# floswald/SMM.jl

Hardware: AMD Instinct MI355X
Metric: chain-evals/sec (whole node), serialNormal 2p/2m, 4096 chains x 200 iters (higher is better)
Workload: dtype f64

## Files before the change

### smm.jl_amd/csrc/smm_lookahead.hpp

```cpp
#pragma once
__global__ void k_pregen_rng(const KParams P, const int t0, const int W, double* __restrict__ rb) {
    const int N = P.N, np = P.np, TR = P.rb_tries;
    const int Q = (np + 1) / 2;
    const uint32_t per_iter = (uint32_t)TR * (uint32_t)Q * (uint32_t)N;
    const uint32_t i = blockIdx.x * blockDim.x + threadIdx.x;
    if (i >= per_iter) return;
    const int q = (int)(i % (uint32_t)Q);
    const uint32_t rest = i / (uint32_t)Q;
    const int r = (int)(rest % (uint32_t)TR);
    const int c = (int)(rest / (uint32_t)TR);
    const int w = (int)blockIdx.y;
    const int t = t0 + w;
    const uint32_t gc = (uint32_t)(P.offset + c);
    double* blk = rb + ((size_t)w * N + c) * P.RBW;
    if (t > 1) {
        double z0, z1 = 0.0;
        if (P.user_ntab) {
            const size_t base = (((size_t)(t - 1) * TR + r) * np) * N + c;
            z0 = P.user_ntab[base + (size_t)(2 * q) * N];
            if (2 * q + 1 < np) z1 = P.user_ntab[base + (size_t)(2 * q + 1) * N];
        } else {
            rng_prop_normal2(P.seed, gc, (uint32_t)t, (uint32_t)r, (uint32_t)q, z0, z1);
        }
        blk[1 + r * np + 2 * q] = z0;
        if (2 * q + 1 < np) blk[1 + r * np + 2 * q + 1] = z1;
    }
    if (r == 0 && q == 0) blk[0] = P.user_utab ? P.user_utab[(size_t)(t - 1) * N + c] : rng_u(P.seed, gc, (uint32_t)t);
}

__global__ __launch_bounds__(XWG) void k_exch_plan(const KParams P, const int t0, unsigned long long* __restrict__ plan,
                                                   double* __restrict__ plan_mi, uint32_t* __restrict__ lv_pairs,
                                                   double* __restrict__ lv_mi, uint32_t* __restrict__ lv_off,
                                                   uint32_t* __restrict__ lv_pairs_p, uint32_t* __restrict__ lv_offp) {
    extern __shared__ __attribute__((aligned(16))) unsigned char xsm[];
    const int tid = threadIdx.x, lane = tid & 63, wave = tid >> 6;
    const int t = t0 + blockIdx.x;
    const int Ng = P.Ng, K = P.plan_K;
    uint32_t* cnt = (uint32_t*)xsm;
    uint32_t* ep = cnt + Ng + 2;
    uint16_t* pi = (uint16_t*)(ep + 2 * K);
    uint16_t* pj = pi + K;
    uint32_t* wsum = (uint32_t*)(pj + K);
    unsigned long long* out = plan + (size_t)blockIdx.x * K;
    double* out_mi = plan_mi + (size_t)blockIdx.x * K;

    if (P.ts && blockIdx.x == 0 && tid == 0) P.ts[(size_t)8 * 60000 + 80] = wall_clock64();
    for (int c = tid; c < Ng; c += XWG) cnt[c] = 0;
    if (P.pairtab) {
        for (int q = tid; q < K; q += XWG) {
            pi[q] = (uint16_t)P.pairtab[((size_t)(t - 1) * K + q) * 2];
            pj[q] = (uint16_t)P.pairtab[((size_t)(t - 1) * K + q) * 2 + 1];
        }
    } else {
        PairPerm pp;
        pp.init(P.seed, (uint32_t)t, (uint64_t)Ng * (uint64_t)(Ng - 1) / 2);
        for (int q = tid; q < K; q += XWG) {
            int32_t i, j;
            pair_unrank(pp.eval((uint64_t)q), i, j);
            pi[q] = (uint16_t)i;
            pj[q] = (uint16_t)j;
        }
    }
    __syncthreads();
    if (P.ts && blockIdx.x == 0 && tid == 0) P.ts[(size_t)8 * 60000 + 81] = wall_clock64();
    for (int q = tid; q < K; q += XWG) {
        atomicAdd(&cnt[pi[q]], 1u);
        atomicAdd(&cnt[pj[q]], 1u);
    }
    __syncthreads();
    {
        constexpr int PER = XLDS_MAX / XWG;
        const int per = (Ng + XWG - 1) / XWG;
        const int c0 = tid * per;
        uint32_t loc[PER];
        uint32_t sum = 0;
#pragma unroll
        for (int u = 0; u < PER; ++u) {
            const int c = c0 + u;
            const uint32_t v = (u < per && c < Ng) ? cnt[c] : 0u;
            loc[u] = sum;
            sum += v;
        }
        uint32_t incl = sum;
#pragma unroll
        for (int off = 1; off < 64; off <<= 1) {
            const uint32_t o = __shfl_up(incl, off, 64);
            if (lane >= off) incl += o;
        }
        if (lane == 63) wsum[wave] = incl;
        __syncthreads();
        uint32_t base = 0;
        for (int w = 0; w < wave; ++w) base += wsum[w];
        const uint32_t excl = base + incl - sum;
#pragma unroll
        for (int u = 0; u < PER; ++u) {
            const int c = c0 + u;
            if (u < per && c < Ng) cnt[c] = excl + loc[u];
        }
    }
    __syncthreads();
    for (int q = tid; q < K; q += XWG) {
        ep[atomicAdd(&cnt[pi[q]], 1u)] = (uint32_t)q;
        ep[atomicAdd(&cnt[pj[q]], 1u)] = (uint32_t)q;
    }
    __syncthreads();
    constexpr int MAXPP = XLDS_MAX / XWG;
    uint16_t rri[MAXPP], rrj[MAXPP];
#pragma unroll
    for (int m = 0; m < MAXPP; ++m) {
        const int q = tid + m * XWG;
        rri[m] = 0; rrj[m] = 0;
        if (q < K) {
            const uint32_t i = pi[q], j = pj[q];
            uint32_t b = i ? cnt[i - 1] : 0u, e = cnt[i], ri = 0, rj = 0;
            for (uint32_t x = b; x < e; ++x) ri += (ep[x] < (uint32_t)q) ? 1u : 0u;
            b = j ? cnt[j - 1] : 0u; e = cnt[j];
            for (uint32_t x = b; x < e; ++x) rj += (ep[x] < (uint32_t)q) ? 1u : 0u;
            out[q] = (unsigned long long)i | ((unsigned long long)j << 16) | ((unsigned long long)ri << 32) |
                     ((unsigned long long)rj << 48);
            out_mi[q] = P.min_improve_g[i];
            rri[m] = (uint16_t)ri; rrj[m] = (uint16_t)rj;
        }
    }
    __syncthreads();
    if (P.ts && blockIdx.x == 0 && tid == 0) P.ts[(size_t)8 * 60000 + 82] = wall_clock64();
#pragma unroll
    for (int m = 0; m < MAXPP; ++m) {
        const int q = tid + m * XWG;
        if (q < K) {
            const uint32_t i = pi[q], j = pj[q];
            ep[(i ? cnt[i - 1] : 0u) + rri[m]] = (uint32_t)q;
            ep[(j ? cnt[j - 1] : 0u) + rrj[m]] = (uint32_t)q;
        }
    }
    __syncthreads();
    int prei[MAXPP], prej[MAXPP];
    bool lasti[MAXPP], lastj[MAXPP];
#pragma unroll
    for (int m = 0; m < MAXPP; ++m) {
        const int q = tid + m * XWG;
        prei[m] = -1; prej[m] = -1; lasti[m] = false; lastj[m] = false;
        if (q < K) {
            const uint32_t i = pi[q], j = pj[q];
            if (rri[m]) prei[m] = (int)ep[(i ? cnt[i - 1] : 0u) + rri[m] - 1];
            if (rrj[m]) prej[m] = (int)ep[(j ? cnt[j - 1] : 0u) + rrj[m] - 1];
            lasti[m] = (i ? cnt[i - 1] : 0u) + rri[m] + 1u == cnt[i];
            lastj[m] = (j ? cnt[j - 1] : 0u) + rrj[m] + 1u == cnt[j];
        }
    }
    __syncthreads();
    uint16_t* lvl = (uint16_t*)ep;
    uint16_t* lvl_b = lvl + K;
    uint32_t* lhist = cnt;
    for (int q = tid; q < K; q += XWG) { lvl[q] = 0; lvl_b[q] = 0; }
    __syncthreads();
    {
        uint16_t own[MAXPP];
#pragma unroll
        for (int m = 0; m < MAXPP; ++m) own[m] = 0;
        const uint16_t* cur = lvl;
        uint16_t* nxt = lvl_b;
        int changed = 1;
        while (changed) {
            int mine = 0;
#pragma unroll
            for (int m = 0; m < MAXPP; ++m) {
                const int q = tid + m * XWG;
                if (q < K) {
                    const uint32_t a = prei[m] >= 0 ? cur[prei[m]] : 0u, b = prej[m] >= 0 ? cur[prej[m]] : 0u;
                    const bool known = (prei[m] < 0 || a) && (prej[m] < 0 || b);
                    const uint16_t nl = known ? (uint16_t)(1u + (a > b ? a : b)) : (uint16_t)0;
                    if (nl != own[m]) mine = 1;
                    own[m] = nl;
                    nxt[q] = nl;
                }
            }
            changed = __syncthreads_or(mine);
            const uint16_t* x = cur; cur = nxt; nxt = (uint16_t*)x;
        }
    }
    if (P.ts && blockIdx.x == 0 && tid == 0) P.ts[(size_t)8 * 60000 + 83] = wall_clock64();
    for (int c = tid; c < Ng + 2; c += XWG) lhist[c] = 0;
    __syncthreads();
    for (int q = tid; q < K; q += XWG) atomicAdd(&lhist[lvl[q]], 1u);
    __syncthreads();
    uint32_t* wsum2 = wsum + 16;
    __shared__ uint32_t s_nlev;
    if (tid == 0) s_nlev = 0;
    __syncthreads();
    {
        uint32_t mx = 0;
        for (int q = tid; q < K; q += XWG) mx = lvl[q] > mx ? lvl[q] : mx;
        atomicMax(&s_nlev, mx);
    }
    __syncthreads();
    const int nlev = (int)s_nlev;
    {
        constexpr int PER = XLDS_MAX / XWG + 1;
        const int n = nlev + 1;
        const int per = (n + XWG - 1) / XWG;
        const int c0 = tid * per;
        uint32_t loc[PER];
        uint32_t sum = 0;
#pragma unroll
        for (int u = 0; u < PER; ++u) {
            const int c = c0 + u;
            const uint32_t v = (u < per && c < n) ? lhist[c] : 0u;
            loc[u] = sum;
            sum += v;
        }
        uint32_t incl = sum;
#pragma unroll
        for (int off = 1; off < 64; off <<= 1) {
            const uint32_t o = __shfl_up(incl, off, 64);
            if (lane >= off) incl += o;
        }
        if (lane == 63) wsum2[wave] = incl;
        __syncthreads();
        uint32_t base = 0;
        for (int w = 0; w < wave; ++w) base += wsum2[w];
        const uint32_t excl = base + incl - sum;
#pragma unroll
        for (int u = 0; u < PER; ++u) {
            const int c = c0 + u;
            if (u < per && c < n) lhist[c] = excl + loc[u];
        }
    }
    __syncthreads();
    uint32_t* o_off = lv_off + (size_t)blockIdx.x * (K + 2);
    for (int l = tid; l < nlev; l += XWG) o_off[l] = (l + 2 <= nlev) ? lhist[l + 2] : (uint32_t)K;
    if (tid == 0) o_off[K + 1] = (uint32_t)nlev;
    __shared__ uint32_t s_lst[LV_MAXLEV + 2], s_pst[LV_MAXLEV + 2];
    const bool lean = lv_pairs_p != nullptr && nlev <= LV_MAXLEV;
    uint32_t* o_pp = lv_pairs_p ? lv_pairs_p + (size_t)blockIdx.x * P.plan_Kp : nullptr;
    if (lv_offp && tid == 0) {
        uint32_t* o = lv_offp + (size_t)blockIdx.x * LV_OFFP;
        o[33] = (uint32_t)nlev; o[34] = lean ? 1u : 0u;
        if (lean) {
            uint32_t acc = 0;
            for (int c = 1; c <= nlev; ++c) {
                s_lst[c] = lhist[c]; s_pst[c] = acc; o[c - 1] = acc;
                acc += ((c + 1 <= nlev ? lhist[c + 1] : (uint32_t)K) - lhist[c] + 63u) & ~63u;
            }
            s_pst[nlev + 1] = acc; o[nlev] = acc;
        }
    }
    __syncthreads();
    const uint32_t sc8 = (uint32_t)P.lean_unit;
    if (lean) {
        const uint32_t Ng4 = (uint32_t)((Ng + 3) & ~3);
        const uint32_t dummy = P.lean_wide ? (sc8 * Ng4) * 0x10001u : (sc8 * Ng4) | ((sc8 * (Ng4 + 1u)) << 16);
        for (uint32_t q = tid; q < s_pst[nlev + 1]; q += XWG) o_pp[q] = dummy;
    }
    __syncthreads();
    uint32_t* o_pairs = lv_pairs + (size_t)blockIdx.x * K;
    double* o_mi = lv_mi + (size_t)blockIdx.x * K;
    uint16_t ci[MAXPP], cj[MAXPP], lvq[MAXPP];
#pragma unroll
    for (int m = 0; m < MAXPP; ++m) {
        const int q = tid + m * XWG;
        ci[m] = 0; cj[m] = 0; lvq[m] = 0;
        if (q < K) {
            const uint32_t lv = lvl[q];
            const uint32_t pos = atomicAdd(&lhist[lv], 1u);
            const uint32_t i = pi[q], j = pj[q];
            o_pairs[pos] = i | (j << 16);
            o_mi[pos] = P.min_improve_g[i];
            if (lean) o_pp[s_pst[lv] + (pos - s_lst[lv])] = (sc8 * i) | ((sc8 * j) << 16);
            ci[m] = (uint16_t)i; cj[m] = (uint16_t)j; lvq[m] = (uint16_t)lv;
        }
    }
    if (P.ts && blockIdx.x == 0 && tid == 0) P.ts[(size_t)8 * 60000 + 84] = wall_clock64();
    if (P.cone_ok == nullptr) return;
    const int tiles = P.cone_tiles;
    uint32_t* o_ok = (uint32_t*)P.cone_ok + blockIdx.x;
    if (!lean) {
        if (tid == 0) *o_ok = 0u;
        return;
    }
    const int LS = nlev + 1;
    int wpp = (int)(((size_t)150 * 1024) / ((size_t)K * 4 + (size_t)32 * LS * 4 + 32 * 4));
    if (wpp > (tiles + 31) / 32) wpp = (tiles + 31) / 32;
    if (wpp < 1) { if (tid == 0) *o_ok = 0u; return; }
    __shared__ uint32_t s_bad;
    if (tid == 0) s_bad = 0u;
    uint32_t* need = (uint32_t*)xsm;
    uint32_t* lcnt = need + (size_t)K * wpp;
    uint32_t* gcnt = lcnt + (size_t)32 * wpp * LS;
    uint16_t* o_gl = P.cone_gather ? P.cone_gather + (size_t)blockIdx.x * tiles * CONE_GCAP : nullptr;
    uint32_t* o_hdr = (uint32_t*)P.cone_hdr + (size_t)blockIdx.x * tiles * CONE_HDRW;
    uint32_t* o_cp = (uint32_t*)P.cone_pairs + (size_t)blockIdx.x * tiles * (CONE_LEVELS * 64);
    const uint32_t ct = (uint32_t)P.cone_ct;
    for (int b0 = 0; b0 < tiles; b0 += 32 * wpp) {
        const int nb = min(32 * wpp, tiles - b0);
        __syncthreads();
        for (int x = tid; x < K * wpp + 32 * wpp * LS + 32 * wpp; x += XWG) need[x] = 0u;
        __syncthreads();
        auto seed = [&](const uint32_t c, const int q) {
            const uint32_t b = (c - (uint32_t)P.offset) / ct - (uint32_t)b0;
            if (b < (uint32_t)nb) atomicOr(&need[(size_t)q * wpp + (b >> 5)], 1u << (b & 31u));
        };
#pragma unroll
        for (int m = 0; m < MAXPP; ++m) {
            const int q = tid + m * XWG;
            if (q < K) {
                if (lasti[m]) seed(ci[m], q);
                if (lastj[m]) seed(cj[m], q);
            }
        }
        if (P.ts && blockIdx.x == 0 && tid == 0) P.ts[(size_t)8 * 60000 + 85] = wall_clock64();
        __syncthreads();
        for (int l = nlev; l >= 2; --l) {
#pragma unroll
            for (int m = 0; m < MAXPP; ++m) {
                const int q = tid + m * XWG;
                if (q < K && lvq[m] == l) {
                    uint32_t* ri = prei[m] >= 0 ? &need[(size_t)prei[m] * wpp] : nullptr;
                    uint32_t* rj = prej[m] >= 0 ? &need[(size_t)prej[m] * wpp] : nullptr;
                    if ((wpp & 3) == 0) {
                        for (int w = 0; w < wpp; w += 8) {
                            const uint4 v0 = *(const uint4*)&need[(size_t)q * wpp + w];
                            const uint4 v1 = w + 4 < wpp ? *(const uint4*)&need[(size_t)q * wpp + w + 4] : make_uint4(0u, 0u, 0u, 0u);
                            const uint32_t v[8] = {v0.x, v0.y, v0.z, v0.w, v1.x, v1.y, v1.z, v1.w};
#pragma unroll
                            for (int x = 0; x < 8; ++x)
                                if (v[x]) {
                                    if (ri) atomicOr(&ri[w + x], v[x]);
                                    if (rj) atomicOr(&rj[w + x], v[x]);
                                }
                        }
                    } else
                        for (int w = 0; w < wpp; ++w) {
                            const uint32_t v = need[(size_t)q * wpp + w];
                            if (v) {
                                if (ri) atomicOr(&ri[w], v);
                                if (rj) atomicOr(&rj[w], v);
                            }
                        }
                }
            }
            __syncthreads();
        }
        if (P.ts && blockIdx.x == 0 && tid == 0) P.ts[(size_t)8 * 60000 + 86] = wall_clock64();
#pragma unroll
        for (int m = 0; m < MAXPP; ++m) {
            const int q = tid + m * XWG;
            if (q < K)
                for (int w = 0; w < wpp; ++w) {
                    uint32_t bits = need[(size_t)q * wpp + w];
                    while (bits) {
                        const uint32_t b = (uint32_t)w * 32u + (uint32_t)__builtin_ctz(bits);
                        bits &= bits - 1u;
                        atomicAdd(&lcnt[b * LS + lvq[m]], 1u);
                    }
                }
        }
        __syncthreads();
        if (P.ts && blockIdx.x == 0 && tid == 0) P.ts[(size_t)8 * 60000 + 87] = wall_clock64();
        for (int b = tid; b < nb; b += XWG) {
            uint32_t sub = 0;
            uint32_t hw[CONE_HDRW];
#pragma unroll
            for (int x = 0; x < CONE_HDRW; ++x) hw[x] = 0u;
            for (int l = 1; l <= nlev; ++l) {
                const uint32_t n = lcnt[b * LS + l];
                lcnt[b * LS + l] = sub * 64u;
                for (uint32_t x = 0; x < n; x += 64u, ++sub)
                    if (sub < (uint32_t)CONE_LEVELS) {
                        const uint32_t cnt_s = n - x < 64u ? n - x : 64u;
#pragma unroll
                        for (int y = 0; y < CONE_LEVELS / 4; ++y)
                            if ((int)(sub >> 2) == y) hw[1 + y] |= cnt_s << (8u * (sub & 3u));
                    }
            }
            hw[0] = sub < (uint32_t)CONE_LEVELS ? sub : (uint32_t)CONE_LEVELS;
            if (sub > (uint32_t)CONE_LEVELS) atomicOr(&s_bad, 1u);
#pragma unroll
            for (int x = 0; x < CONE_HDRW; ++x) o_hdr[(size_t)(b0 + b) * CONE_HDRW + x] = hw[x];
        }
        __syncthreads();
        if (P.ts && blockIdx.x == 0 && tid == 0) P.ts[(size_t)8 * 60000 + 88] = wall_clock64();
#pragma unroll
        for (int m = 0; m < MAXPP; ++m) {
            const int q = tid + m * XWG;
            if (q < K) {
                const uint32_t word = (sc8 * ci[m]) | ((sc8 * cj[m]) << 16);
                const bool gi = o_gl && rri[m] == 0, gj = o_gl && rrj[m] == 0;
                const uint32_t ti = ((uint32_t)ci[m] - (uint32_t)P.offset) / ct, tj = ((uint32_t)cj[m] - (uint32_t)P.offset) / ct;
                for (int w = 0; w < wpp; ++w) {
                    uint32_t bits = need[(size_t)q * wpp + w];
                    while (bits) {
                        uint32_t bb[4], dst[4], g1[4], g2[4];
#pragma unroll
                        for (int u = 0; u < 4; ++u) {
                            bb[u] = 0xffffffffu;
                            if (bits) { bb[u] = (uint32_t)w * 32u + (uint32_t)__builtin_ctz(bits); bits &= bits - 1u; }
                        }
#pragma unroll
                        for (int u = 0; u < 4; ++u) {
                            dst[u] = 0u; g1[u] = 0xffffffffu; g2[u] = 0xffffffffu;
                            if (bb[u] != 0xffffffffu) {
                                dst[u] = atomicAdd(&lcnt[bb[u] * LS + lvq[m]], 1u);
                                if (gi && ti != (uint32_t)b0 + bb[u]) g1[u] = atomicAdd(&gcnt[bb[u]], 1u);
                                if (gj && tj != (uint32_t)b0 + bb[u]) g2[u] = atomicAdd(&gcnt[bb[u]], 1u);
                            }
                        }
#pragma unroll
                        for (int u = 0; u < 4; ++u)
                            if (bb[u] != 0xffffffffu) {
                                if (dst[u] < (uint32_t)(CONE_LEVELS * 64)) o_cp[(size_t)(b0 + bb[u]) * (CONE_LEVELS * 64) + dst[u]] = word;
                                if (g1[u] < (uint32_t)CONE_GCAP) o_gl[(size_t)(b0 + bb[u]) * CONE_GCAP + g1[u]] = ci[m];
                                if (g2[u] < (uint32_t)CONE_GCAP) o_gl[(size_t)(b0 + bb[u]) * CONE_GCAP + g2[u]] = cj[m];
                            }
                    }
                }
            }
        }
        if (o_gl) {
            __syncthreads();
            for (int b = tid; b < nb; b += XWG) {
                const uint32_t g = gcnt[b];
                if (g > (uint32_t)CONE_GCAP) atomicOr(&s_bad, 1u);
                o_hdr[(size_t)(b0 + b) * CONE_HDRW] |= (g < (uint32_t)CONE_GCAP ? g : (uint32_t)CONE_GCAP) << 16;
            }
        }
    }
    __syncthreads();
    if (P.ts && blockIdx.x == 0 && tid == 0) P.ts[(size_t)8 * 60000 + 89] = wall_clock64();
    if (tid == 0) *o_ok = s_bad ? 0u : 1u;
}
__host__ __device__ inline size_t plan_cone_bytes() { return (size_t)152 * 1024; }
```

Baseline: 325.9 million.

## Build cone tile lists by bit-transposed scan instead of per-pair atomics

Reindexes the cone 'need' bitmasks by level-sorted pair position and transposes them, so each tile becomes a contiguous bit row across pairs. A prefix sum over popcounts splits the pairs among thread segments, and each thread walks its tile's bits in order to write level-grouped pair lists and gather lists directly. This replaces the earlier per-pair atomic histogram, header pass and atomic scatter. It also caps words-per-pair at a constant so all tiles fit in a single pass. The cost is more complex shuffle and scan logic and fixed shared-memory layout assumptions enforced by static_asserts.

```diff
diff --git a/smm.jl_amd/csrc/smm_lookahead.hpp b/smm.jl_amd/csrc/smm_lookahead.hpp
--- a/smm.jl_amd/csrc/smm_lookahead.hpp
+++ b/smm.jl_amd/csrc/smm_lookahead.hpp
@@ -28,6 +28,11 @@
     if (r == 0 && q == 0) blk[0] = P.user_utab ? P.user_utab[(size_t)(t - 1) * N + c] : rng_u(P.seed, gc, (uint32_t)t);
 }
 
+constexpr int CONE_WPP = 8;
+__host__ __device__ inline size_t plan_cone_fixed(int Kr) { return (size_t)Kr * 4 + (size_t)(Kr / 32) * 12 + (size_t)XWG * 4 + (size_t)32 * CONE_WPP * 4; }
+__host__ __device__ inline size_t plan_cone_bytes() { return (size_t)152 * 1024; }
+static_assert((size_t)4096 * 4 * CONE_WPP + (size_t)4096 * 4 + 4096 / 32 * 12 + XWG * 4 + 32 * CONE_WPP * 4 <= (size_t)152 * 1024, "4096 pairs: all 256 tiles in one pass");
+static_assert(XLDS_MAX / 32 <= 4 * 64, "one wave sums the position words' bits, four each");
 __global__ __launch_bounds__(XWG) void k_exch_plan(const KParams P, const int t0, unsigned long long* __restrict__ plan,
                                                    double* __restrict__ plan_mi, uint32_t* __restrict__ lv_pairs,
                                                    double* __restrict__ lv_mi, uint32_t* __restrict__ lv_off,
@@ -255,11 +260,11 @@
     __syncthreads();
     uint32_t* o_pairs = lv_pairs + (size_t)blockIdx.x * K;
     double* o_mi = lv_mi + (size_t)blockIdx.x * K;
-    uint16_t ci[MAXPP], cj[MAXPP], lvq[MAXPP];
+    uint16_t ci[MAXPP], cj[MAXPP], lvq[MAXPP], posr[MAXPP];
 #pragma unroll
     for (int m = 0; m < MAXPP; ++m) {
         const int q = tid + m * XWG;
-        ci[m] = 0; cj[m] = 0; lvq[m] = 0;
+        ci[m] = 0; cj[m] = 0; lvq[m] = 0; posr[m] = 0;
         if (q < K) {
             const uint32_t lv = lvl[q];
             const uint32_t pos = atomicAdd(&lhist[lv], 1u);
@@ -267,7 +272,7 @@
             o_pairs[pos] = i | (j << 16);
             o_mi[pos] = P.min_improve_g[i];
             if (lean) o_pp[s_pst[lv] + (pos - s_lst[lv])] = (sc8 * i) | ((sc8 * j) << 16);
-            ci[m] = (uint16_t)i; cj[m] = (uint16_t)j; lvq[m] = (uint16_t)lv;
+            ci[m] = (uint16_t)i; cj[m] = (uint16_t)j; lvq[m] = (uint16_t)lv; posr[m] = (uint16_t)pos;
         }
     }
     if (P.ts && blockIdx.x == 0 && tid == 0) P.ts[(size_t)8 * 60000 + 84] = wall_clock64();
@@ -278,34 +283,66 @@
         if (tid == 0) *o_ok = 0u;
         return;
     }
-    const int LS = nlev + 1;
-    int wpp = (int)(((size_t)150 * 1024) / ((size_t)K * 4 + (size_t)32 * LS * 4 + 32 * 4));
+    const int Kr = K > 0 ? (K + 31) & ~31 : 32, KW = Kr >> 5;
+    int wpp = (int)((plan_cone_bytes() - plan_cone_fixed(Kr)) / ((size_t)Kr * 4));
+    if (wpp > CONE_WPP) wpp = CONE_WPP;
     if (wpp > (tiles + 31) / 32) wpp = (tiles + 31) / 32;
     if (wpp < 1) { if (tid == 0) *o_ok = 0u; return; }
-    __shared__ uint32_t s_bad;
+    __shared__ uint32_t s_bad, s_lend[LV_MAXLEV + 3];
     if (tid == 0) s_bad = 0u;
+    __syncthreads();
+    if (tid <= nlev + 1) s_lend[tid] = tid == 0 ? 0u : tid <= nlev ? lhist[tid] : 0x7fffffffu;
+    __syncthreads();
     uint32_t* need = (uint32_t*)xsm;
-    uint32_t* lcnt = need + (size_t)K * wpp;
-    uint32_t* gcnt = lcnt + (size_t)32 * wpp * LS;
+    uint32_t* pwl = need + (size_t)Kr * wpp;
+    uint32_t* fi = pwl + Kr;
+    uint32_t* fj = fi + KW;
+    uint32_t* pcnt = fj + KW;
+    uint32_t* segt = pcnt + KW;
+    uint32_t* gcnt = segt + XWG;
+    {
+        uint16_t* q2p = (uint16_t*)need;
+        for (int x = tid; x < 2 * KW; x += XWG) fi[x] = 0u;
+#pragma unroll
+        for (int m = 0; m < MAXPP; ++m) {
+            const int q = tid + m * XWG;
+            if (q < K) { pwl[posr[m]] = (sc8 * ci[m]) | ((sc8 * cj[m]) << 16); q2p[q] = posr[m]; }
+        }
+        __syncthreads();
+#pragma unroll
+        for (int m = 0; m < MAXPP; ++m) {
+            const int q = tid + m * XWG;
+            if (q < K) {
+                if (rri[m] == 0) atomicOr(&fi[posr[m] >> 5], 1u << (posr[m] & 31u));
+                if (rrj[m] == 0) atomicOr(&fj[posr[m] >> 5], 1u << (posr[m] & 31u));
+                if (prei[m] >= 0) prei[m] = (int)q2p[prei[m]];
+                if (prej[m] >= 0) prej[m] = (int)q2p[prej[m]];
+            }
+        }
+    }
     uint16_t* o_gl = P.cone_gather ? P.cone_gather + (size_t)blockIdx.x * tiles * CONE_GCAP : nullptr;
     uint32_t* o_hdr = (uint32_t*)P.cone_hdr + (size_t)blockIdx.x * tiles * CONE_HDRW;
     uint32_t* o_cp = (uint32_t*)P.cone_pairs + (size_t)blockIdx.x * tiles * (CONE_LEVELS * 64);
     const uint32_t ct = (uint32_t)P.cone_ct;
-    for (int b0 = 0; b0 < tiles; b0 += 32 * wpp) {
-        const int nb = min(32 * wpp, tiles - b0);
-        __syncthreads();
-        for (int x = tid; x < K * wpp + 32 * wpp * LS + 32 * wpp; x += XWG) need[x] = 0u;
-        __syncthreads();
-        auto seed = [&](const uint32_t c, const int q) {
+    const int TP = 32 * wpp, NSEG = XWG / TP;
+    const int seg = tid / TP, bt = tid - seg * TP;
+    for (int b0 = 0; b0 < tiles; b0 += TP) {
+        const int nb = min(TP, tiles - b0);
+        __syncthreads();
+        for (int x = tid; x < Kr * wpp; x += XWG) need[x] = 0u;
+        for (int x = tid; x < TP; x += XWG) gcnt[x] = 0u;
+        for (int x = tid; x < nb * CONE_HDRW; x += XWG) o_hdr[(size_t)b0 * CONE_HDRW + x] = 0u;
+        __syncthreads();
+        auto seed = [&](const uint32_t c, const uint32_t pos) {
             const uint32_t b = (c - (uint32_t)P.offset) / ct - (uint32_t)b0;
-            if (b < (uint32_t)nb) atomicOr(&need[(size_t)q * wpp + (b >> 5)], 1u << (b & 31u));
+            if (b < (uint32_t)nb) atomicOr(&need[(size_t)pos * wpp + (b >> 5)], 1u << (b & 31u));
         };
 #pragma unroll
         for (int m = 0; m < MAXPP; ++m) {
             const int q = tid + m * XWG;
             if (q < K) {
-                if (lasti[m]) seed(ci[m], q);
-                if (lastj[m]) seed(cj[m], q);
+                if (lasti[m]) seed(ci[m], posr[m]);
+                if (lastj[m]) seed(cj[m], posr[m]);
             }
         }
         if (P.ts && blockIdx.x == 0 && tid == 0) P.ts[(size_t)8 * 60000 + 85] = wall_clock64();
@@ -315,12 +352,13 @@
             for (int m = 0; m < MAXPP; ++m) {
                 const int q = tid + m * XWG;
                 if (q < K && lvq[m] == l) {
+                    const uint32_t* rq = &need[(size_t)posr[m] * wpp];
                     uint32_t* ri = prei[m] >= 0 ? &need[(size_t)prei[m] * wpp] : nullptr;
                     uint32_t* rj = prej[m] >= 0 ? &need[(size_t)prej[m] * wpp] : nullptr;
                     if ((wpp & 3) == 0) {
                         for (int w = 0; w < wpp; w += 8) {
-                            const uint4 v0 = *(const uint4*)&need[(size_t)q * wpp + w];
-                            const uint4 v1 = w + 4 < wpp ? *(const uint4*)&need[(size_t)q * wpp + w + 4] : make_uint4(0u, 0u, 0u, 0u);
+                            const uint4 v0 = *(const uint4*)&rq[w];
+                            const uint4 v1 = w + 4 < wpp ? *(const uint4*)&rq[w + 4] : make_uint4(0u, 0u, 0u, 0u);
                             const uint32_t v[8] = {v0.x, v0.y, v0.z, v0.w, v1.x, v1.y, v1.z, v1.w};
 #pragma unroll
                             for (int x = 0; x < 8; ++x)
@@ -331,7 +369,7 @@
                         }
                     } else
                         for (int w = 0; w < wpp; ++w) {
-                            const uint32_t v = need[(size_t)q * wpp + w];
+                            const uint32_t v = rq[w];
                             if (v) {
                                 if (ri) atomicOr(&ri[w], v);
                                 if (rj) atomicOr(&rj[w], v);
@@ -342,91 +380,183 @@
             __syncthreads();
         }
         if (P.ts && blockIdx.x == 0 && tid == 0) P.ts[(size_t)8 * 60000 + 86] = wall_clock64();
-#pragma unroll
-        for (int m = 0; m < MAXPP; ++m) {
-            const int q = tid + m * XWG;
-            if (q < K)
-                for (int w = 0; w < wpp; ++w) {
-                    uint32_t bits = need[(size_t)q * wpp + w];
-                    while (bits) {
-                        const uint32_t b = (uint32_t)w * 32u + (uint32_t)__builtin_ctz(bits);
-                        bits &= bits - 1u;
-                        atomicAdd(&lcnt[b * LS + lvq[m]], 1u);
+        for (int c0 = 0; c0 < KW; c0 += 2 * (XWG / 64)) {
+            const int pw = c0 + 2 * wave + (lane >> 5), r = lane & 31;
+            const bool on = pw < KW;
+            uint32_t v[CONE_WPP];
+            uint32_t pc = 0u;
+#pragma unroll
+            for (int w = 0; w < CONE_WPP; ++w) v[w] = 0u;
+            if (on) {
+                const uint32_t* row = &need[(size_t)(pw * 32 + r) * wpp];
+                if ((wpp & 3) == 0) {
+#pragma unroll
+                    for (int w = 0; w < CONE_WPP; w += 4)
+                        if (w < wpp) {
+                            const uint4 t4 = *(const uint4*)&row[w];
+                            v[w] = t4.x; v[w + 1] = t4.y; v[w + 2] = t4.z; v[w + 3] = t4.w;
+                        }
+                } else {
+#pragma unroll
+                    for (int w = 0; w < CONE_WPP; ++w)
+                        if (w < wpp) v[w] = row[w];
+                }
+            }
+#pragma unroll
+            for (int w = 0; w < CONE_WPP; ++w) pc += (uint32_t)__builtin_popcount(v[w]);
+#pragma unroll
+            for (int w = 0; w < CONE_WPP; ++w)
+                if (w < wpp) {
+#pragma unroll
+                    for (int e = 4; e >= 0; --e) {
+                        const int j = 1 << e;
+                        const uint32_t mk = j == 16 ? 0x0000ffffu : j == 8 ? 0x00ff00ffu : j == 4 ? 0x0f0f0f0fu : j == 2 ? 0x33333333u : 0x55555555u;
+                        const uint32_t keep = (r & j) ? ~mk : mk, rot = (r & j) ? (uint32_t)j : (uint32_t)(32 - j);
+                        const uint32_t p = (uint32_t)__shfl_xor((int)v[w], j, 64);
+                        v[w] = (v[w] & keep) | (__builtin_amdgcn_alignbit(p, p, rot) & ~keep);
                     }
                 }
+#pragma unroll
+            for (int e = 4; e >= 0; --e) pc += (uint32_t)__shfl_xor((int)pc, 1 << e, 64);
+            __syncthreads();
+            if (on) {
+#pragma unroll
+                for (int w = 0; w < CONE_WPP; ++w)
+                    if (w < wpp) need[(size_t)pw * TP + 32 * w + r] = v[w];
+                if (r == 0) pcnt[pw] = pc;
+            }
+        }
+        __syncthreads();
+        if (wave == 0) {
+            constexpr int PER = XLDS_MAX / 32 / 64;
+            uint32_t loc[PER], sum = 0u;
+#pragma unroll
+            for (int u = 0; u < PER; ++u) {
+                const int c = lane * PER + u;
+                sum += c < KW ? pcnt[c] : 0u;
+                loc[u] = sum;
+            }
+            uint32_t incl = sum;
+#pragma unroll
+            for (int o = 1; o < 64; o <<= 1) {
+                const uint32_t x = __shfl_up(incl, o, 64);
+                if (lane >= o) incl += x;
+            }
+#pragma unroll
+            for (int u = 0; u < PER; ++u) {
+                const int c = lane * PER + u;
+                if (c < KW) pcnt[c] = incl - sum + loc[u];
+            }
         }
         __syncthreads();
         if (P.ts && blockIdx.x == 0 && tid == 0) P.ts[(size_t)8 * 60000 + 87] = wall_clock64();
-        for (int b = tid; b < nb; b += XWG) {
-            uint32_t sub = 0;
-            uint32_t hw[CONE_HDRW];
-#pragma unroll
-            for (int x = 0; x < CONE_HDRW; ++x) hw[x] = 0u;
-            for (int l = 1; l <= nlev; ++l) {
-                const uint32_t n = lcnt[b * LS + l];
-                lcnt[b * LS + l] = sub * 64u;
-                for (uint32_t x = 0; x < n; x += 64u, ++sub)
-                    if (sub < (uint32_t)CONE_LEVELS) {
-                        const uint32_t cnt_s = n - x < 64u ? n - x : 64u;
-#pragma unroll
-                        for (int y = 0; y < CONE_LEVELS / 4; ++y)
-                            if ((int)(sub >> 2) == y) hw[1 + y] |= cnt_s << (8u * (sub & 3u));
+        const bool active = seg < NSEG && bt < nb;
+        int w0 = 0, w1 = 0;
+        uint32_t lv0 = 1u;
+        if (active) {
+            const uint32_t total = pcnt[KW - 1];
+            auto bound = [&](const int s) {
+                if (s <= 0) return 0;
+                if (s >= NSEG) return KW;
+                const uint32_t thr = (total * (uint32_t)s + (uint32_t)NSEG - 1u) / (uint32_t)NSEG;
+                int lo = 0, hi = KW;
+                while (lo < hi) {
+                    const int mid = (lo + hi) >> 1;
+                    if (pcnt[mid] >= thr) hi = mid; else lo = mid + 1;
+                }
+                return lo;
+            };
+            w0 = bound(seg); w1 = bound(seg + 1);
+            while ((int)lv0 < nlev && s_lend[lv0] < (uint32_t)w0 * 32u) ++lv0;
+            uint32_t off = 0u, c0 = 0u, hasb = 0u, lv = lv0, nbp = s_lend[lv0];
+            for (int pw = w0; pw < w1; ++pw) {
+                uint32_t bits = need[(size_t)pw * TP + bt];
+                const uint32_t p0 = (uint32_t)pw * 32u;
+                for (;;) {
+                    const uint32_t lim = nbp - p0;
+                    if (lim >= 32u) { off += (uint32_t)__builtin_popcount(bits); break; }
+                    const uint32_t low = (1u << lim) - 1u;
+                    off += (uint32_t)__builtin_popcount(bits & low);
+                    bits &= ~low;
+                    if (!hasb) { c0 = off; hasb = 1u; off = 0u; } else off = (off + 63u) & ~63u;
+                    ++lv; nbp = s_lend[lv];
+                }
+            }
+            if (!hasb) { c0 = off; off = 0u; }
+            segt[tid] = c0 | (off << 14) | (hasb << 31);
+        }
+        __syncthreads();
+        uint32_t off = 0u;
+        if (active) {
+            for (int s = 0; s < seg; ++s) {
+                const uint32_t e = segt[s * TP + bt];
+                off += e & 0x3fffu;
+                if (e >> 31) off = ((off + 63u) & ~63u) + ((e >> 14) & 0x1ffffu);
+            }
+        }
+        if (P.ts && blockIdx.x == 0 && tid == 0) P.ts[(size_t)8 * 60000 + 88] = wall_clock64();
+        if (active) {
+            unsigned char* o_cnt = (unsigned char*)(o_hdr + (size_t)(b0 + bt) * CONE_HDRW + 1);
+            auto setbyte = [&](const uint32_t s, const uint32_t n) { o_cnt[s] = (unsigned char)n; };
+            uint32_t run = off;
+            auto flush = [&]() {
+                const uint32_t e = (off >> 6) < (uint32_t)CONE_LEVELS ? (off >> 6) : (uint32_t)CONE_LEVELS;
+                for (uint32_t s = run >> 6; s < e; ++s) setbyte(s, 64u);
+                run = off & ~63u;
+            };
+            auto close = [&]() {
+                flush();
+                const uint32_t rem = off & 63u;
+                if (rem) {
+                    if ((off >> 6) < (uint32_t)CONE_LEVELS) setbyte(off >> 6, rem);
+                    off = (off | 63u) + 1u;
+                }
+                run = off;
+            };
+            uint32_t* o_cp_t = o_cp + (size_t)(b0 + bt) * (CONE_LEVELS * 64);
+            uint16_t* o_gl_t = o_gl ? o_gl + (size_t)(b0 + bt) * CONE_GCAP : nullptr;
+            const uint32_t own0 = sc8 * ((uint32_t)P.offset + (uint32_t)(b0 + bt) * ct), ownn = sc8 * ct, sh = 31u - (uint32_t)__builtin_clz(sc8);
+            auto gather = [&](uint32_t g, const uint32_t p0, const uint32_t half) {
+                while (g) {
+                    const uint32_t k = (uint32_t)__builtin_ctz(g);
+                    g &= g - 1u;
+                    const uint32_t c = (pwl[p0 + k] >> half) & 0xffffu;
+                    if (c - own0 >= ownn) {
+                        const uint32_t n = atomicAdd(&gcnt[bt], 1u);
+                        if (n < (uint32_t)CONE_GCAP) o_gl_t[n] = (uint16_t)(c >> sh);
                     }
-            }
-            hw[0] = sub < (uint32_t)CONE_LEVELS ? sub : (uint32_t)CONE_LEVELS;
-            if (sub > (uint32_t)CONE_LEVELS) atomicOr(&s_bad, 1u);
-#pragma unroll
-            for (int x = 0; x < CONE_HDRW; ++x) o_hdr[(size_t)(b0 + b) * CONE_HDRW + x] = hw[x];
-        }
-        __syncthreads();
-        if (P.ts && blockIdx.x == 0 && tid == 0) P.ts[(size_t)8 * 60000 + 88] = wall_clock64();
-#pragma unroll
-        for (int m = 0; m < MAXPP; ++m) {
-            const int q = tid + m * XWG;
-            if (q < K) {
-                const uint32_t word = (sc8 * ci[m]) | ((sc8 * cj[m]) << 16);
-                const bool gi = o_gl && rri[m] == 0, gj = o_gl && rrj[m] == 0;
-                const uint32_t ti = ((uint32_t)ci[m] - (uint32_t)P.offset) / ct, tj = ((uint32_t)cj[m] - (uint32_t)P.offset) / ct;
-                for (int w = 0; w < wpp; ++w) {
-                    uint32_t bits = need[(size_t)q * wpp + w];
-                    while (bits) {
-                        uint32_t bb[4], dst[4], g1[4], g2[4];
-#pragma unroll
-                        for (int u = 0; u < 4; ++u) {
-                            bb[u] = 0xffffffffu;
-                            if (bits) { bb[u] = (uint32_t)w * 32u + (uint32_t)__builtin_ctz(bits); bits &= bits - 1u; }
-                        }
-#pragma unroll
-                        for (int u = 0; u < 4; ++u) {
-                            dst[u] = 0u; g1[u] = 0xffffffffu; g2[u] = 0xffffffffu;
-                            if (bb[u] != 0xffffffffu) {
-                                dst[u] = atomicAdd(&lcnt[bb[u] * LS + lvq[m]], 1u);
-                                if (gi && ti != (uint32_t)b0 + bb[u]) g1[u] = atomicAdd(&gcnt[bb[u]], 1u);
-                                if (gj && tj != (uint32_t)b0 + bb[u]) g2[u] = atomicAdd(&gcnt[bb[u]], 1u);
-                            }
-                        }
-#pragma unroll
-                        for (int u = 0; u < 4; ++u)
-                            if (bb[u] != 0xffffffffu) {
-                                if (dst[u] < (uint32_t)(CONE_LEVELS * 64)) o_cp[(size_t)(b0 + bb[u]) * (CONE_LEVELS * 64) + dst[u]] = word;
-                                if (g1[u] < (uint32_t)CONE_GCAP) o_gl[(size_t)(b0 + bb[u]) * CONE_GCAP + g1[u]] = ci[m];
-                                if (g2[u] < (uint32_t)CONE_GCAP) o_gl[(size_t)(b0 + bb[u]) * CONE_GCAP + g2[u]] = cj[m];
-                            }
+                }
+            };
+            uint32_t lv = lv0, nbp = s_lend[lv0];
+            for (int pw = w0; pw < w1; ++pw) {
+                uint32_t bits = need[(size_t)pw * TP + bt];
+                const uint32_t p0 = (uint32_t)pw * 32u;
+                if (o_gl_t) { gather(bits & fi[pw], p0, 0u); gather(bits & fj[pw], p0, 16u); }
+                for (;;) {
+                    const uint32_t lim = nbp - p0;
+                    uint32_t part = lim >= 32u ? bits : bits & ((1u << lim) - 1u);
+                    bits ^= part;
+                    while (part) {
+                        const uint32_t k = (uint32_t)__builtin_ctz(part);
+                        part &= part - 1u;
+                        if (off < (uint32_t)(CONE_LEVELS * 64)) o_cp_t[off] = pwl[p0 + k];
+                        ++off;
                     }
-                }
-            }
-        }
-        if (o_gl) {
-            __syncthreads();
-            for (int b = tid; b < nb; b += XWG) {
-                const uint32_t g = gcnt[b];
-                if (g > (uint32_t)CONE_GCAP) atomicOr(&s_bad, 1u);
-                o_hdr[(size_t)(b0 + b) * CONE_HDRW] |= (g < (uint32_t)CONE_GCAP ? g : (uint32_t)CONE_GCAP) << 16;
-            }
+                    if (lim >= 32u) break;
+                    close();
+                    ++lv; nbp = s_lend[lv];
+                }
+            }
+            if (seg == NSEG - 1) close(); else flush();
+        }
+        __syncthreads();
+        if (active && seg == NSEG - 1) {
+            const uint32_t sub = off >> 6, g = o_gl ? gcnt[bt] : 0u;
+            if (sub > (uint32_t)CONE_LEVELS || g > (uint32_t)CONE_GCAP) atomicOr(&s_bad, 1u);
+            o_hdr[(size_t)(b0 + bt) * CONE_HDRW] = (sub < (uint32_t)CONE_LEVELS ? sub : (uint32_t)CONE_LEVELS) | ((g < (uint32_t)CONE_GCAP ? g : (uint32_t)CONE_GCAP) << 16);
         }
     }
     __syncthreads();
     if (P.ts && blockIdx.x == 0 && tid == 0) P.ts[(size_t)8 * 60000 + 89] = wall_clock64();
     if (tid == 0) *o_ok = s_bad ? 0u : 1u;
 }
-__host__ __device__ inline size_t plan_cone_bytes() { return (size_t)152 * 1024; }
```

After: 323.9 million. Within noise of the previous version (-0.6%).
